# uga-ssrl/SSRLCV

Hardware: AMD Instinct MI355X
Metric: Mpix/s SIFT extract (+ Mmatches/s 128-D brute-force, see `matcher`) (higher is better)
Workload: dtype f32; 1 GPU; 2-view 4096x4096 pair per GPU (tools/scene.py pinhole views (PCG32 terrain + texture through Image::Camera)): SIFT_FeatureFactory::generateFeatures (sparse DoG path) on each image, pixels resident in HBM; images_per_gpu=2, parallelism=image-pair shard, library=release build (libssrlcv_hip_release.so)

## Files before the change

ssrlcv_amd/capi.py:

```python
import ctypes

import numpy as np
import torch

from . import _lib

LIB = _lib.load()

c_u32, c_f32, c_vp, c_sz, c_int = ctypes.c_uint32, ctypes.c_float, ctypes.c_void_p, ctypes.c_size_t, ctypes.c_int

OUT_DMATCH, OUT_UINT2_PAIR, OUT_MATCH = 0, 1, 2
_OUT_SIZE = {OUT_DMATCH: 48, OUT_UINT2_PAIR: 16, OUT_MATCH: 40}


class SsrlcvError(RuntimeError):
    pass


class MalformedPairList(SsrlcvError):
    """the device merge's input status word: an index out of range or a query matched twice in one pair"""


def check(rc):
    if rc != 0:
# ... 442 lines not shown


def math_eval(fn, a, b=None):
    a_d = torch.from_numpy(np.ascontiguousarray(a, dtype=np.float32)).cuda()
    b_d = None if b is None else torch.from_numpy(np.ascontiguousarray(b, dtype=np.float32)).cuda()
    out = torch.empty_like(a_d)
    check(LIB.ssrlcv_hip_math_eval(c_int(fn), ptr(a_d), ptr(b_d), ptr(out), c_sz(a_d.numel()), stream_ptr()))
    return out.cpu().numpy()


class SiftPlan:

    def __init__(self, w, h, max_orientations=2, orientation_threshold=0.8, orientation_contrib_width=1.5,
                 descriptor_contrib_width=6.0, max_keypoints_per_octave=0, alloc=True):
        self.w, self.h = w, h
        p = SiftParams(max_orientations, orientation_threshold, orientation_contrib_width, descriptor_contrib_width,
                       max_keypoints_per_octave)
        self.handle = c_vp()
        check(LIB.ssrlcv_sift_plan_create(c_u32(w), c_u32(h), ctypes.byref(p), ctypes.byref(self.handle)))
        self.workspace_bytes = LIB.ssrlcv_sift_plan_workspace_bytes(self.handle)
        self.max_features = LIB.ssrlcv_sift_plan_max_features(self.handle)
        self.workspace = dev_bytes(self.workspace_bytes) if alloc else None
        self.features = dev_bytes(self.max_features * 152) if alloc else None
        self.num_features = torch.zeros(1, dtype=torch.int32, device="cuda") if alloc else None

    def __del__(self):
        if getattr(self, "handle", None) and LIB is not None:
            LIB.ssrlcv_sift_plan_destroy(self.handle)
            self.handle = None

    def set_stop_stage(self, stage):
        LIB.ssrlcv_sift_plan_set_stop_stage(self.handle, c_int(stage))

    def set_stage_event(self, event):
        handle = None
        if event is not None:
            event.record()
            handle = event.cuda_event
        self._stage_event = event
        check(LIB.ssrlcv_sift_plan_set_stage_event(self.handle, c_vp(handle) if handle is not None else None))

    def build_dog(self, pixels_d):
        check(LIB.ssrlcv_hip_sift_build_dog(self.handle, ptr(pixels_d), ptr(self.workspace), stream_ptr()))

    def describe(self):
        check(LIB.ssrlcv_hip_sift_describe(self.handle, ptr(self.workspace), ptr(self.features),
                                           ptr(self.num_features), stream_ptr()))

    def stage(self, stage):
        check(LIB.ssrlcv_hip_sift_stage(self.handle, ptr(self.workspace), c_int(stage), ptr(self.features),
                                        ptr(self.num_features), stream_ptr()))

    def extract(self, pixels_d):
        check(LIB.ssrlcv_hip_sift_extract(self.handle, ptr(pixels_d), ptr(self.workspace), ptr(self.features),
                                          ptr(self.num_features), stream_ptr()))

    def count(self):
        mask = c_u32(0)
        rc = LIB.ssrlcv_sift_plan_overflow(self.handle, ptr(self.workspace), ctypes.byref(mask), stream_ptr())
        if mask.value:
            raise SsrlcvError("key-point capacity exceeded in octaves %s" % [o for o in range(4) if mask.value >> o & 1])
        check(rc)
        return int(self.num_features.item())

    def overflow_mask(self):
        mask = c_u32(0)
        LIB.ssrlcv_sift_plan_overflow(self.handle, ptr(self.workspace), ctypes.byref(mask), stream_ptr())
        return mask.value

    def level(self, kind, octave, blur):
        data, mm = c_vp(), c_vp()
        w, h = c_u32(), c_u32()
        check(LIB.ssrlcv_sift_plan_level(self.handle, ptr(self.workspace), c_int(kind), c_int(octave), c_int(blur),
                                         ctypes.byref(data), ctypes.byref(w), ctypes.byref(h), ctypes.byref(mm)))
        torch.cuda.synchronize()
        base = self.workspace.data_ptr()
        off = data.value - base
        n = w.value * h.value
        lvl = self.workspace[off: off + 4 * n].view(torch.float32).cpu().numpy().reshape(h.value, w.value).copy()
        moff = mm.value - base
        mmv = self.workspace[moff: moff + 8].view(torch.float32).cpu().numpy().copy()
        return lvl, (float(mmv[0]), float(mmv[1]))

    def keypoints(self, octave, dtype):
        lst, idx = c_vp(), c_vp()
        check(LIB.ssrlcv_sift_plan_keypoints(self.handle, ptr(self.workspace), c_int(octave), ctypes.byref(lst),
                                             ctypes.byref(idx)))
        torch.cuda.synchronize()
        base = self.workspace.data_ptr()
        ioff = idx.value - base
        state = self.workspace[ioff: ioff + 32].view(torch.int32).cpu().numpy().copy()
        n = int(state[5]) if int(state[6]) else 0
        loff = lst.value - base
        kps = to_host(self.workspace[loff: loff + 32 * max(n, 1)], dtype, n)
        return kps, state[:6].copy(), int(state[7])

    def features_host(self, dtype):
        n = self.count()
        return to_host(self.features[: 152 * max(n, 1)], dtype, n)
```

ssrlcv_amd/csrc/keypoints.hip:

```cpp
#include <hip/hip_runtime.h>
#include <float.h>
#include <math.h>
#include <stdlib.h>
#include "compact.h"
#include "dev_switch.h"
#include "scan_lookback.h"
#include "device_math.h"
#include "sift_plan.h"
#include "ssrlcv_hip.h"

using svp::OctaveState;

namespace {

struct LevelSet {
  const float* lvl[svp::kGauss];
  const float* lvlMinMax;
  const float* minmax;
  const float2* polar;
  int w, h;
};

struct DogView {
  const float* lo;
// ... 168 lines not shown
  float hess[3][3], hinv[3][3] = {{0.0f, 0.0f, 0.0f}, {0.0f, 0.0f, 0.0f}, {0.0f, 0.0f, 0.0f}};
  float grad[3], temp[3], offset[3] = {0.0f, 0.0f, 0.0f};
  int bl = kp.blur;
  for (int attempt = 0; attempt < 5; ++attempt) {
    const auto Dl = src.view(bl - 1), Dm = src.view(bl), Du = src.view(bl + 1);
#define PM(yy, xx) Dm.norm((size_t)(yy) * W + (xx))
#define PL(yy, xx) Dl.norm((size_t)(yy) * W + (xx))
#define PU(yy, xx) Du.norm((size_t)(yy) * W + (xx))
    grad[0] = PM(ly, lx + 1) - PM(ly, lx - 1);
    grad[1] = PM(ly + 1, lx) - PM(ly - 1, lx);
    grad[2] = PU(ly, lx) - PL(ly, lx);
    float centre = PM(ly, lx);
    hess[0][0] = grad[0] - 2 * centre;
    hess[0][1] = (PM(ly + 1, lx + 1) - PM(ly - 1, lx + 1) - PM(ly + 1, lx - 1) + PM(ly - 1, lx - 1)) / 4.0f;
    hess[0][2] = (PU(ly, lx + 1) - PL(ly, lx + 1) - PU(ly, lx - 1) + PL(ly, lx - 1)) / 4.0f;
    hess[1][0] = hess[0][1];
    hess[1][1] = grad[1] - 2 * centre;
    hess[1][2] = (PU(ly + 1, lx) - PL(ly + 1, lx) - PU(ly - 1, lx) + PL(ly - 1, lx)) / 4.0f;
    hess[2][0] = hess[0][2];
    hess[2][1] = hess[1][2];
    hess[2][2] = grad[2] - 2 * centre;
#pragma unroll
    for (int r = 0; r < 3; ++r)
#pragma unroll
      for (int c = 0; c < 3; ++c) hess[r][c] *= -1.0f;
    sv::inverse3(hess, hinv);
#pragma unroll
    for (int r = 0; r < 3; ++r) {
      float val = 0;
#pragma unroll
      for (int c = 0; c < 3; ++c) val = __builtin_fmaf(hinv[r][c], grad[c], val);
      offset[r] = val;
    }
#pragma unroll
    for (int c = 0; c < 3; ++c) {
      float val = 0;
#pragma unroll
      for (int r = 0; r < 3; ++r) val = __builtin_fmaf(hess[r][c], grad[r], val);
      temp[c] = val;
    }
    if (fabsf(offset[0]) <= 0.5f && fabsf(offset[1]) <= 0.5f && fabsf(offset[2]) <= 0.5f) {
      kp.loc.x = (float)lx + offset[0];
      kp.loc.y = (float)ly + offset[1];
      lx = (int)roundf(kp.loc.x);
      ly = (int)roundf(kp.loc.y);
      kp.discard = (uint8_t)(lx <= 0 || ly <= 0 || lx >= W - 1 || ly >= H - 1);
      if (kp.discard) break;
      kp.intensity = PM(ly, lx) - (0.5f * ((temp[0] * grad[0]) + (temp[1] * grad[1]) + (temp[2] * grad[2])));
      kp.sigma = sigmaMin * sv_powf(mult, ((float)bl + offset[2]));
      if (fabsf(offset[2]) > 0.5) bl += (offset[2] > 0) ? 1 : -1;
      break;
    } else if (attempt == 4) {
      kp.discard = 1;
      break;
    } else {
      if (fabsf(offset[0]) > 0.5) lx += (offset[0] > 0) ? 1 : -1;
      if (fabsf(offset[1]) > 0.5) ly += (offset[1] > 0) ? 1 : -1;
      kp.loc.x = (float)lx;
      kp.loc.y = (float)ly;
      if (fabsf(offset[2]) > 0.5) bl += (offset[2] > 0) ? 1 : -1;
      if (bl >= numBlurs - 1 || bl <= 0 || lx <= 0 || ly <= 0 || lx >= W - 1 || ly >= H - 1) {
        kp.discard = 1;
        break;
      }
    }
#undef PM
#undef PL
#undef PU
  }
  kp.blur = bl;
}

__global__ __launch_bounds__(256) void k_refine(const OctaveState* st, ssrlcv_sskeypoint* kps, LevelSet L, float sigmaMin,
                                                float mult) {
  int n = st->hasExtrema ? st->n : 0;
  const PlanSource src{L};
  for (int gi = blockIdx.x * 256 + threadIdx.x; gi < n; gi += gridDim.x * 256) {
    ssrlcv_sskeypoint kp = kps[gi];
    refine_one(kp, L.w, L.h, svp::kDog, sigmaMin, mult, src);
    kps[gi] = kp;
  }
}

constexpr int kPolRows = 16;
struct PolarJobs {
  LevelSet L[svp::kOctaves];
  float2* out[svp::kOctaves];
  uint32_t start[svp::kOctaves + 1];
  uint32_t tilesX[svp::kOctaves];
};
#ifndef SSRLCV_NT_STORES
#define SSRLCV_NT_STORES 1
#endif
typedef float f32x2p __attribute__((ext_vector_type(2)));
__device__ __forceinline__ float polar_ld(const float* p) {
#if SSRLCV_NT_STORES
  return __builtin_nontemporal_load(p);
#else
  return *p;
#endif
}
__global__ __launch_bounds__(256) void k_polar(PolarJobs jobs) {
  __shared__ float s_n[kPolRows][256 + 2];
  int o = 0;
#pragma unroll
  for (int k = 1; k < svp::kOctaves; ++k)
    if (blockIdx.x >= jobs.start[k]) o = k;
  const LevelSet& L = jobs.L[o];
  float2* __restrict__ out = jobs.out[o];
  const uint32_t tile = blockIdx.x - jobs.start[o];
  const int tileX = (int)(tile % jobs.tilesX[o]), tileY = (int)(tile / jobs.tilesX[o]);
  const int W = L.w, H = L.h;
  const int x0 = tileX * 256, y0 = tileY * kPolRows;
  const int t = threadIdx.x, x = x0 + t;
  const int xc = x < W ? x : W - 1;
  const bool haloRole = t < 2 * kPolRows;
  const int hside = t & 1;
  int hx = hside ? x0 + 256 : x0 - 1;
  hx = hx < 0 ? 0 : (hx > W - 1 ? W - 1 : hx);
  int hy = y0 + (t >> 1);
  hy = hy > H - 1 ? H - 1 : hy;
  size_t rowOff[kPolRows + 2];
#pragma unroll
  for (int j = 0; j < kPolRows + 2; ++j) {
    int yy = y0 - 1 + j;
    yy = yy < 0 ? 0 : (yy > H - 1 ? H - 1 : yy);
    rowOff[j] = (size_t)yy * W + xc;
  }
  const size_t haloOff = (size_t)hy * W + hx;
  float nlo[kPolRows + 2], nloH = 0.0f;
  {
    const float mn = L.lvlMinMax[2];
    const sv::Divisor rg = sv::make_divisor(L.lvlMinMax[3] - mn);
    const float* __restrict__ g = L.lvl[1];
#pragma unroll
    for (int j = 0; j < kPolRows + 2; ++j) nlo[j] = sv::div_by(polar_ld(g + rowOff[j]) - mn, rg);
    if (haloRole) nloH = sv::div_by(g[haloOff] - mn, rg);
  }
  const int cl = x == 0 ? 1 : (x == W - 1 ? t - 1 : t);
  const int cr = x == 0 ? 3 : (x == W - 1 ? t + 1 : t + 2);
#pragma unroll 1
  for (int lvl = 1; lvl <= 3; ++lvl) {
    const float mn = L.lvlMinMax[2 * (lvl + 1)];
    const sv::Divisor rg = sv::make_divisor(L.lvlMinMax[2 * (lvl + 1) + 1] - mn);
    const float dmn = L.minmax[2 * lvl];
    const sv::Divisor drg = sv::make_divisor(L.minmax[2 * lvl + 1] - dmn);
    const float* __restrict__ g = L.lvl[lvl + 1];
    float v[kPolRows + 2];
#pragma unroll
    for (int j = 0; j < kPolRows + 2; ++j) {
      const float nhi = sv::div_by(polar_ld(g + rowOff[j]) - mn, rg);
      v[j] = sv::div_by((nhi - nlo[j]) - dmn, drg);
      nlo[j] = nhi;
    }
    if (lvl > 1) __syncthreads();
#pragma unroll
    for (int i = 0; i < kPolRows; ++i) s_n[i][t + 1] = v[i + 1];
    if (haloRole) {
      const float nhi = sv::div_by(g[haloOff] - mn, rg);
      s_n[t >> 1][hside ? 257 : 0] = sv::div_by((nhi - nloH) - dmn, drg);
      nloH = nhi;
    }
    __syncthreads();
    float2* __restrict__ lvlOut = out + (size_t)(lvl - 1) * svp::polar_level_stride(W, H);
    if (tile == 0) {
      if (t == 0) lvlOut[0] = make_float2(0.0f, 0.0f);
      for (int i = t; i < W + 1; i += 256) lvlOut[1 + (size_t)W * H + i] = make_float2(0.0f, 0.0f);
    }
    if (x < W) {
      float2* __restrict__ o = lvlOut + 1 + (size_t)y0 * W + x;
#pragma unroll
      for (int i = 0; i < kPolRows; ++i) {
        const int y = y0 + i;
        if (y >= H) break;
        float2 g2;
        g2.x = s_n[i][cr] - s_n[i][cl];
        const float up = y == 0 ? v[i + 3 < kPolRows + 2 ? i + 3 : kPolRows + 1] : (y == H - 1 ? v[i + 1] : v[i + 2]);
        const float dn = y == 0 ? v[i + 1] : (y == H - 1 ? v[i > 0 ? i - 1 : 0] : v[i]);
        g2.y = up - dn;
        float2 r;
        r.x = sqrtf((g2.x * g2.x) + (g2.y * g2.y));
        r.y = sv_atan2f(g2.y, g2.x);
#if SSRLCV_NT_STORES
        __builtin_nontemporal_store(f32x2p{r.x, r.y}, reinterpret_cast<f32x2p*>(o + (size_t)i * W));
#else
        o[(size_t)i * W] = r;
#endif
      }
    }
  }
}
typedef float f32x2 __attribute__((ext_vector_type(2)));
__device__ __forceinline__ int round_pos(float v) {
  int r;
  asm("v_cvt_rpi_i32_f32 %0, %1" : "=v"(r) : "v"(v));
  return r;
}

__device__ __forceinline__ float fmod_2pi_above(float v, float p) { return v >= p ? v - p : v; }
__device__ __forceinline__ float2 polar_px(const float2* __restrict__ pl, int W, int x, int y) {
  return pl[y * W + x];
}
__device__ __forceinline__ int round_coord(float v) {
  int r;
  asm("v_cvt_rpi_i32_f32 %0, %1" : "=v"(r) : "v"(v));
  return v == -0.5f ? -1 : r;
}

constexpr int kThetaChunk = 8;

struct RangeTable {
  uint32_t first[20], count[20], start[20];
  uint32_t total;
  uint32_t pad[3];
};
static_assert(sizeof(RangeTable) == 256, "tables sit at 256-byte strides in the plan's group block");
__device__ __constant__ const int kSegOrder[5] = {3, 2, 1, 4, 0};
__device__ __forceinline__ void build_ranges(const OctaveState* st, RangeTable* tab, int unitShift, uint32_t sel) {
  uint32_t pos = 0;
  for (int k = 0; k < 5; ++k) {
    const int seg = kSegOrder[k];
    for (int o = 0; o < svp::kOctaves; ++o) {
      const int r = k * 4 + o;
      uint32_t first = 0, count = 0;
      if (st[o].hasExtrema && ((sel >> (o * 5 + seg)) & 1u)) {
        const int lo = st[o].idx[seg], hi = seg < svp::kDog - 1 ? st[o].idx[seg + 1] : st[o].n;
        if (hi > lo) { first = (uint32_t)lo; count = (uint32_t)(hi - lo); }
      }
      tab->first[r] = first;
      tab->count[r] = count;
      tab->start[r] = pos;
      pos += (count + (1u << unitShift) - 1) >> unitShift;
    }
  }
  tab->total = pos;
}
__global__ void k_build_ranges(const OctaveState* st, RangeTable* tab, int unitShift, uint32_t sel) { build_ranges(st, tab, unitShift, sel); }
__global__ void k_book_and_desc_ranges(OctaveState* st, uint32_t* featBase, uint32_t* numFeatures, uint32_t maxFeatures, RangeTable* tab) {
  uint32_t tot = 0;
  for (int o = 0; o < svp::kOctaves; ++o) {
    featBase[o] = tot;
    tot += st[o].hasExtrema ? (uint32_t)st[o].n : 0u;
  }
  if (tot > maxFeatures) tot = maxFeatures;
  *numFeatures = tot;
  build_ranges(st, tab, 0, 0xFFFFFu);
}

constexpr int kOct0Groups = svp::kSampleGroups - 1;
struct GroupCtl {
  uint32_t segStart[svp::kDog];
  uint32_t totals[svp::kSampleGroups + 1];
  uint32_t groupSum[svp::kSampleGroups];
  uint32_t done[svp::kSampleGroups];
  uint32_t regular;
  uint32_t cut[2];
  uint32_t pad[32 - svp::kDog - 3 * svp::kSampleGroups - 4];
};
static_assert(sizeof(GroupCtl) == 128, "four of them + eight range tables fit the plan's 4 KB group block");
__device__ __forceinline__ bool blur_indices_regular(const OctaveState* st) {
  if (!st->hasExtrema) return true;
  bool ok = st->idx[0] == 0;
  for (int k = 1; k < svp::kDog; ++k) ok = ok && st->idx[k - 1] <= st->idx[k];
  return ok && st->idx[svp::kDog - 1] <= st->n;
}
__global__ void k_build_group_ranges(const OctaveState* st, RangeTable* tabs, GroupCtl* ctl, int unitShift, bool forceIrregular) {
  const bool reg = blur_indices_regular(st) && !forceIrregular;
  const uint32_t n0 = st[0].hasExtrema && st[0].n > 0 ? (uint32_t)st[0].n : 0u;
  ctl[0].regular = reg ? 1u : 0u;
  ctl[0].cut[0] = reg && n0 ? (uint32_t)st[0].idx[2] : n0;
  ctl[0].cut[1] = reg && n0 ? (uint32_t)st[0].idx[3] : n0;
  const uint32_t oct0 = 0x1Fu, rest = 0xFFFFFu & ~oct0;
// ... 37 lines not shown
  int r = 0;
#pragma unroll
  for (int k = 1; k < 20; ++k)
    if (tab->start[k] <= u) r = k;
  return r;
}

struct OctaveSet {
  LevelSet L[svp::kOctaves];
  const ssrlcv_sskeypoint* kps[svp::kOctaves];
  float pixelWidth[svp::kOctaves];
  float* thetas[svp::kOctaves];
  uint32_t* thetaCnt[svp::kOctaves];
  const void* consts[svp::kOctaves];
};

template <int MAXO, int LPKS>
__global__ __launch_bounds__(64) void k_thetas(const OctaveState* states, const RangeTable* tab, OctaveSet set, float lambda,
                                               float orientationThreshold) {
  constexpr int LANES = 1 << LPKS, PER_BLOCK = 64 >> LPKS, CW = kThetaChunk * LANES;
  __shared__ float s_hist[36][PER_BLOCK];
  if (blockIdx.x >= tab->total) return;
  const int range = __builtin_amdgcn_readfirstlane(range_of(tab, blockIdx.x));
  const int octave = range & 3, useg = kSegOrder[range >> 2];
  const LevelSet& L = set.L[octave];
  const float pixelWidth = set.pixelWidth[octave];
  const int t = threadIdx.x, sub = t & (LANES - 1), col = t >> LPKS;
  const float fsub2 = (float)(2 * sub);
  const uint32_t local = (blockIdx.x - tab->start[range]) * PER_BLOCK + (uint32_t)(t >> LPKS);
  const bool have = local < tab->count[range];
  const int gi = (int)(tab->first[range] + local);
  const float pi = SSRLCV_PI_F;
  const float rad10 = pi / 18.0f;
  const float inv10 = 1.0f / rad10;
  ssrlcv_sskeypoint kp;
  kp.loc.x = kp.loc.y = 0.0f;
  kp.sigma = 1.0f;
  if (have) kp = set.kps[octave][gi];
  const float kx = kp.loc.x, ky = kp.loc.y;
  const float windowWidth = ceilf(kp.sigma * 3.0f * lambda / pixelWidth);
  const float minx = kx - windowWidth, miny = ky - windowWidth, maxx = kx + windowWidth, maxy = ky + windowWidth;
  const bool inside = have && useg >= 1 && useg <= 3 &&
                      !(minx < 0.0f || miny < 0.0f || maxx >= (unsigned)(L.w - 1) || maxy >= (unsigned)(L.h - 1));
#pragma unroll
  for (int i = 0; i < 36 * PER_BLOCK / 64; ++i) (&s_hist[0][0])[i * 64 + t] = 0.0f;
  const float weight = 2.0f * lambda * lambda * kp.sigma * kp.sigma;
  const float rweight = 1.0f / weight;
  const int W = L.w;
  const size_t levelStride = svp::polar_level_stride(L.w, L.h);
  {
    const float2* base = L.polar + (size_t)(useg - 1) * levelStride;
    const __amdgpu_buffer_rsrc_t rsrc = __builtin_amdgcn_make_buffer_rsrc((void*)base, 0, (int)(uint32_t)(levelStride * 8), 0x00020000);
    typedef unsigned u32x4 __attribute__((ext_vector_type(4)));
    typedef unsigned u32x2 __attribute__((ext_vector_type(2)));
    struct Cursor { float x, y, ty2; unsigned rowoff; bool act; };
    Cursor cf;
    cf.x = minx;
    cf.y = miny;
    cf.ty2 = (miny - ky) * (miny - ky);
    cf.rowoff = (unsigned)round_pos(miny) * (unsigned)W + 1u;
    cf.act = inside;
    auto advance = [&](Cursor& c) {
      float xn = c.x + (float)CW;
      if (__any(c.act && !(c.x >= (float)CW))) {
        float ch = c.x;
#pragma unroll 8
        for (int i = 0; i < CW; ++i) ch += 1.0f;
        xn = c.x >= (float)CW ? xn : ch;
      }
      if (c.act) {
        if (xn <= maxx) {
          c.x = xn;
        } else {
          c.x = minx;
          c.y += 1.0f;
          if (!(c.y <= maxy)) c.act = false;
          const float ty = c.y - ky;
          c.ty2 = ty * ty;
          c.rowoff = (unsigned)round_pos(c.y) * (unsigned)W + 1u;
        }
      }
    };
    typedef u32x4 Chunk[kThetaChunk / 2];
    auto fetch = [&](const Cursor& c, Chunk& into) {
      if (!c.act) return;
      const unsigned off = (c.rowoff + (unsigned)round_pos(c.x)) * 8u + 16u * (unsigned)sub;
#pragma unroll
      for (int j = 0; j < kThetaChunk / 4; ++j) into[j] = __builtin_amdgcn_raw_buffer_load_b128(rsrc, (int)(off + 16u * LANES * j), 0, 0);
    };
    auto fetch_upper = [&](const Cursor& c, Chunk& into) {
      if (!c.act) return;
      const unsigned off = (c.rowoff + (unsigned)round_pos(c.x)) * 8u + 16u * (unsigned)sub;
#pragma unroll
      for (int j = kThetaChunk / 4; j < kThetaChunk / 2; ++j) into[j] = __builtin_amdgcn_raw_buffer_load_b128(rsrc, (int)(off + 16u * LANES * j), 0, 0);
    };
    auto wants_upper = [&](const Cursor& c) { return __any(c.act && c.x + (float)(CW / 2 - 1) <= maxx); };
    Chunk qa, qb;
    Cursor ca, cb;
#pragma unroll
    for (int j = 0; j < kThetaChunk / 2; ++j) qa[j] = qb[j] = u32x4{0u, 0u, 0u, 0u};
    ca = cf;
    fetch(cf, qa);
    if (wants_upper(cf)) fetch_upper(cf, qa);
    advance(cf);
    cb = cf;
    auto step = [&](Chunk& cur, const Cursor& cc, Chunk& nxt, Cursor& cn) __attribute__((always_inline)) {
      cn = cf;
      fetch(cf, nxt);
      if (wants_upper(cf)) fetch_upper(cf, nxt);
      advance(cf);
      float xs[kThetaChunk];
      float xlast = cc.x + (float)(CW - 1);
#pragma unroll
      for (int i = 0; i < kThetaChunk; ++i) xs[i] = cc.x + (fsub2 + (float)(((i >> 1) << (1 + LPKS)) | (i & 1)));
      if (__any(cc.act && !(cc.x >= (float)CW))) {
        float ch = cc.x;
        float xc[kThetaChunk];
#pragma unroll
        for (int sIdx = 0; sIdx < CW; ++sIdx) {
          const int q = (sIdx >> 1) & (LANES - 1), i = ((sIdx >> (1 + LPKS)) << 1) | (sIdx & 1);
          if (LANES == 1 || q == 0) xc[i] = ch;
          else xc[i] = sub == q ? ch : xc[i];
          if (sIdx + 1 < CW) ch += 1.0f;
        }
        const bool direct = cc.x >= (float)CW;
#pragma unroll
        for (int i = 0; i < kThetaChunk; ++i) xs[i] = direct ? xs[i] : xc[i];
        xlast = direct ? xlast : ch;
      }
      const float cty2 = cc.ty2;
      const unsigned crow = cc.rowoff;
      const bool cact = cc.act;
      const bool aligned = cc.x >= 4.0f && round_pos(xlast) == round_pos(cc.x) + (CW - 1);
      if (__any(cact && !aligned)) {
        if (cact && !aligned) {
#pragma unroll
          for (int i = 0; i < kThetaChunk; ++i) {
            u32x2 e = u32x2{0u, 0u};
            if (xs[i] <= maxx) e = __builtin_amdgcn_raw_buffer_load_b64(rsrc, (int)((crow + (unsigned)round_pos(xs[i])) * 8u), 0, 0);
            cur[i >> 1][(i & 1) * 2] = e[0];
            cur[i >> 1][(i & 1) * 2 + 1] = e[1];
          }
        }
      }
      auto weigh = [&](float ang, float xi, float& wgt, int& bin) {
        const float angle = fmod_2pi_above(ang + (2.0f * pi), 2.0f * pi);
        bin = (int)floorf(sv::exact_div3(angle, rad10, inv10));
        const float tx = xi - kx;
        wgt = sv::expf_nonpos(sv::exact_div5(-((tx * tx) + cty2), weight, rweight));
      };
      const bool upperHalf = __any(cact && xs[kThetaChunk / 2] <= maxx);
      float wg[kThetaChunk], mg[kThetaChunk];
      float* slot[kThetaChunk];
      auto weigh_half = [&](auto hc) __attribute__((always_inline)) {
        constexpr int i0 = decltype(hc)::value * (kThetaChunk / 2);
#pragma unroll
        for (int i = i0; i < i0 + kThetaChunk / 2; ++i) {
          const unsigned um = cur[i >> 1][(i & 1) * 2], ua = cur[i >> 1][(i & 1) * 2 + 1];
          int bin;
          weigh(__builtin_bit_cast(float, ua), xs[i], wg[i], bin);
          const bool counts = cact && xs[i] <= maxx && (unsigned)bin < 36u;
          slot[i] = &s_hist[counts ? bin : 0][col];
          mg[i] = counts ? __builtin_bit_cast(float, um) : 0.0f;
        }
      };
      auto vote_half = [&](auto hc) __attribute__((always_inline)) {
        constexpr int j0 = decltype(hc)::value * (kThetaChunk / 4);
#pragma unroll
        for (int j = j0; j < j0 + kThetaChunk / 4; ++j) {
#pragma unroll
          for (int q = 0; q < LANES; ++q) {
            if (LANES == 1 || sub == q) {
              const float h0 = *slot[2 * j], h1 = *slot[2 * j + 1];
              const float n0 = fmaf(mg[2 * j], wg[2 * j], h0);
              const float n1 = fmaf(mg[2 * j + 1], wg[2 * j + 1], slot[2 * j + 1] == slot[2 * j] ? n0 : h1);
              *slot[2 * j] = n0;
              *slot[2 * j + 1] = n1;
            }
// ... 246 lines not shown
          const float mmag = m == 0 ? magA : m == 1 ? magB : m == 2 ? magC : magD;
#pragma unroll 1
          for (int cell = 0; cell < 16; ++cell) {
            const int ci = lane & 15;
            (void)ci;
            const float hx0 = ((float)(cell >> 2) * 0.5f - 0.75f) * windowWidth, hy0 = ((float)(cell & 3) * 0.5f - 0.75f) * windowWidth;
            const float rx = (hx0 * c) + (hy0 * s), ry = (-hx0 * s) + (hy0 * c);
            float hx = fabsf(rx - mcx), hy = fabsf(ry - mcy);
            if (hx <= binWidth && hy <= binWidth) {
              hx = hx / binWidth;
              hy = hy / binWidth;
              for (int k = 0; k < 8; ++k) {
                float angle = fabsf(mang - ((float)k * rad45));
                if (angle < rad45) {
                  angle /= rad45;
                  const float temp = (1.0f - hx) * (1.0f - hy) * (1.0f - angle) * mmag;
                  atomicAdd(bins + (cell * 8 + k) * kDescCopies + copy, vote_u32(temp));
                }
              }
            }
          }
        }
      }
    }
    __builtin_amdgcn_wave_barrier();
    unsigned t0 = 0u, t1 = 0u;
#pragma unroll
    for (int cpy = 0; cpy < kDescCopies; ++cpy) {
      t0 += bins[lane * kDescCopies + cpy];
      t1 += bins[(lane + 64) * kDescCopies + cpy];
    }
    float v0 = (float)t0, v1 = (float)t1;
    float sq = sqrtf(sv::wave_sum((v0 * v0) + (v1 * v1)));
    v0 = v0 / sq;
    v1 = v1 / sq;
    if (v0 > 0.2f) v0 = 0.2f;
    if (v1 > 0.2f) v1 = 0.2f;
    sq = sqrtf(sv::wave_sum((v0 * v0) + (v1 * v1)));
    {
      int b0 = lane, b1 = lane + 64;
      int o0 = (((b0 >> 3) & 3) * 4 + (b0 >> 5)) * 8 + (b0 & 7);
      int o1 = (((b1 >> 3) & 3) * 4 + (b1 >> 5)) * 8 + (b1 & 7);
      s_bytes[wave][o0] = (uint8_t)roundf(255.0f * v0 / sq);
      s_bytes[wave][o1] = (uint8_t)roundf(255.0f * v1 / sq);
    }
    __builtin_amdgcn_wave_barrier();
    const uint32_t fi = featBase[octave] + (uint32_t)gi;
    if (fi < maxFeatures) {
      ssrlcv_sift_feature* f = features + fi;
      if (lane < 16) *reinterpret_cast<uint2*>(&f->values[lane * 8]) = *reinterpret_cast<const uint2*>(&s_bytes[wave][lane * 8]);
      if (lane == 16) {
        f->parent = -1;
        reinterpret_cast<int*>(f)[1] = 0;
        f->theta = kp.theta;
        f->sigma = kp.sigma;
        f->loc.x = kp.loc.x * pixelWidth;
        f->loc.y = kp.loc.y * pixelWidth;
      }
    }
    __builtin_amdgcn_wave_barrier();
  }
}

LevelSet make_levels(const ssrlcv_sift_plan* plan, char* ws, int o) {
  LevelSet L;
  const svp::OctavePlan& oc = plan->oct[o];
  for (int b = 0; b < svp::kGauss; ++b) L.lvl[b] = (const float*)(ws + plan->off_gauss[o][b]);
  L.lvlMinMax = (const float*)(ws + plan->off_minmax) + (size_t)o * 2 * (svp::kGauss + svp::kDog);
  L.minmax = L.lvlMinMax + 2 * svp::kGauss;
  L.polar = (const float2*)(ws + oc.off_polar);
  L.w = (int)oc.w;
  L.h = (int)oc.h;
  return L;
}

void launch_polar(const ssrlcv_sift_plan* plan, char* ws, hipStream_t st, int oFirst = 0, int oLast = svp::kOctaves - 1) {
  PolarJobs jobs;
  uint32_t pos = 0;
  for (int o = 0; o < svp::kOctaves; ++o) {
    const svp::OctavePlan& oc = plan->oct[o];
    jobs.L[o] = make_levels(plan, ws, o);
    jobs.out[o] = (float2*)(ws + oc.off_polar);
    jobs.start[o] = pos;
    jobs.tilesX[o] = (oc.w + 255) / 256;
    if (o >= oFirst && o <= oLast) pos += jobs.tilesX[o] * ((oc.h + kPolRows - 1) / kPolRows);
  }
  jobs.start[svp::kOctaves] = pos;
  hipLaunchKernelGGL(k_polar, dim3(pos), dim3(256), 0, st, jobs);
}

}
namespace svp {
void launch_polar_octave(const ssrlcv_sift_plan* plan, char* ws, int octave, hipStream_t st) {
  PolarJobs jobs;
  const svp::OctavePlan& oc = plan->oct[octave];
  const uint32_t tilesX = (oc.w + 255) / 256, tiles = tilesX * ((oc.h + kPolRows - 1) / kPolRows);
  for (int o = 0; o < svp::kOctaves; ++o) {
    jobs.L[o] = make_levels(plan, ws, octave);
    jobs.out[o] = (float2*)(ws + oc.off_polar);
    jobs.tilesX[o] = tilesX;
    jobs.start[o] = o <= octave ? 0u : tiles;
  }
  jobs.start[svp::kOctaves] = tiles;
  hipLaunchKernelGGL(k_polar, dim3(tiles), dim3(256), 0, st, jobs);
}
}
namespace {
hipError_t run_discard(OctaveState* st, const ssrlcv_sskeypoint* src, ssrlcv_sskeypoint* dst, uint32_t cap,
                       uint32_t* words, hipStream_t stream) {
  const OctaveState* cst = st;
  auto keyfn = [=] __device__(uint32_t i) -> uint32_t {
    if (!cst->hasExtrema || (int)i >= cst->n) return 0u;
    if (src[i].discard) return 0u;
    return 1u << segment_of(cst, (int)i);
  };
  auto emit = [=] __device__(uint32_t i, int, uint32_t d) { dst[d] = src[i]; };
  uint32_t* totals = nullptr;
  auto post = [=] __device__(const uint32_t* tot) { book_discard(st, tot); };
  return svc::partition<svp::kDog, 8>(cap, keyfn, emit, words, &totals, stream, &st->n, 1u, post);
}

constexpr unsigned kWaveKernelOversubscription = 16;
inline unsigned list_blocks(uint32_t cap) {
  unsigned b = (cap + 255) / 256;
  return b > 1024 ? 1024 : b;
}

}

extern "C" {

int ssrlcv_sift_plan_keypoints(const ssrlcv_sift_plan* plan, void* workspace, int octave, ssrlcv_sskeypoint** list,
                               int** blurIndices_dev) {
  if (!plan || !workspace || octave < 0 || octave >= svp::kOctaves) return SSRLCV_ERR_INVALID_ARG;
  char* ws = (char*)workspace;
  if (list) *list = (ssrlcv_sskeypoint*)(ws + (plan->listInB[octave] ? plan->oct[octave].off_kpB : plan->oct[octave].off_kpA));
  if (blurIndices_dev) *blurIndices_dev = (int*)(ws + plan->off_state + sizeof(OctaveState) * octave);
  return SSRLCV_OK;
}

int ssrlcv_sift_plan_overflow(const ssrlcv_sift_plan* plan, const void* workspace, uint32_t* octaveMask,
                              ssrlcv_stream_t stream) {
  if (!plan || !workspace || !octaveMask) return SSRLCV_ERR_INVALID_ARG;
  OctaveState st[svp::kOctaves];
  SSRLCV_HIP_TRY(hipMemcpyAsync(st, (const char*)workspace + plan->off_state, sizeof st, hipMemcpyDeviceToHost,
                                (hipStream_t)stream));
  SSRLCV_HIP_TRY(hipStreamSynchronize((hipStream_t)stream));
  uint32_t m = 0;
  for (int o = 0; o < svp::kOctaves; ++o)
    if (st[o].overflow) m |= 1u << o;
  *octaveMask = m;
  return m ? SSRLCV_ERR_CAPACITY : SSRLCV_OK;
}

}
namespace {

struct ListCtx {
  const ssrlcv_sift_plan* plan;
  const svp::OctavePlan* oc;
  int o;
  hipStream_t s;
  OctaveState* st;
  LevelSet L;
  ssrlcv_sskeypoint *A, *B;
  uint8_t* flags;
  uint32_t* words;
  uint32_t cap;
  ssrlcv_sskeypoint* cur() const { return plan->listInB[o] ? B : A; }
  ssrlcv_sskeypoint* oth() const { return plan->listInB[o] ? A : B; }
  void flip() const { plan->listInB[o] ^= 1; }
};
ListCtx make_ctx(const ssrlcv_sift_plan* plan, char* ws, int o, hipStream_t s) {
  ListCtx c;
  c.plan = plan;
  c.oc = &plan->oct[o];
  c.o = o;
  c.s = s;
  c.st = (OctaveState*)(ws + plan->off_state) + o;
  c.L = make_levels(plan, ws, o);
  c.A = (ssrlcv_sskeypoint*)(ws + c.oc->off_kpA);
  c.B = (ssrlcv_sskeypoint*)(ws + c.oc->off_kpB);
  c.flags = (uint8_t*)(ws + c.oc->off_flags);
  c.words = (uint32_t*)(ws + c.oc->off_part);
  c.cap = c.oc->cap;
  return c;
}
// ... 1070 lines not shown
```

ssrlcv_amd/csrc/pyramid.hip:

```cpp
#include <hip/hip_runtime.h>
#include <map>
#include <mutex>
#include <float.h>
#include <math.h>
#include <new>
#include <stdlib.h>
#include <string.h>
#include "dev_switch.h"
#include "device_math.h"
#include "sift_plan.h"
#include "ssrlcv_hip.h"

namespace {

__device__ __forceinline__ int sym_coord(int i, int l) {
  int ll = 2 * l;
  if (__builtin_expect(i < -ll || i >= ll, 0)) i = (i + ll) % ll;
  if (i < 0) i += ll;
  return (i > l - 1) ? ll - 1 - i : i;
}

__device__ __forceinline__ int mirror_into(int i, int l, int R) {
  if (l < 64) return sym_coord(i, l);
  i = i > l - 1 + R ? l - 1 + R : i;
// ... 1805 lines not shown
    uint32_t cap = params->maxKeyPointsPerOctave ? params->maxKeyPointsPerOctave : (uint32_t)(P / 16);
    if (cap < 4096) cap = 4096;
    oc.cap = cap;
    oc.off_kpA = take((size_t)cap * sizeof(ssrlcv_sskeypoint));
    oc.off_kpB = take((size_t)cap * sizeof(ssrlcv_sskeypoint));
    oc.off_theta = take((size_t)cap * svp::kMaxOrient * sizeof(float));
    oc.off_thetaCnt = take((size_t)cap * sizeof(uint32_t));
    size_t words = (size_t)3 * 4 * ((P + 8191) / 8192) + 16 +
                   (size_t)svp::kDog * 4 * (((size_t)cap * svp::kMaxOrient + 2047) / 2048) + 16;
    oc.off_part = take(words * 4);
    oc.off_featBase = take(256);
    oc.off_descConst = take((size_t)cap * 32);
    maxFeat += cap;
    if (o + 1 < svp::kOctaves) {
      ow /= 2;
      oh /= 2;
      pixelWidth *= 2.0f;
      for (int b = 0; b < svp::kGauss; ++b) sigmas[b] *= mulX;
    }
  }
  p->off_extremaCounts = take(256);
  p->off_dogPartial = take(sizeof(float) * 2 * svp::kDog * svp::kDogMaxWaves * svp::kOctaves);
  p->off_groups = take(4096);
  p->total = off;
  p->maxFeatures = maxFeat;
  *out = p;
  return SSRLCV_OK;
}

void ssrlcv_sift_plan_destroy(ssrlcv_sift_plan* plan) {
  if (!plan) return;
  if (plan->async) {
    svp::PlanAsync* a = plan->async;
    (void)hipEventDestroy(a->fork);
    for (hipEvent_t e : a->join) (void)hipEventDestroy(e);
    for (hipEvent_t e : a->convDone) (void)hipEventDestroy(e);
    for (hipEvent_t e : a->dogDone) (void)hipEventDestroy(e);
    for (hipEvent_t e : a->polarDone) (void)hipEventDestroy(e);
    for (hipEvent_t e : a->binDone) (void)hipEventDestroy(e);
    (void)hipEventDestroy(a->expandFork);
    (void)hipEventDestroy(a->groupFork);
    for (hipEvent_t e : a->groupExpanded) (void)hipEventDestroy(e);
    for (hipEvent_t e : a->groupReady) (void)hipEventDestroy(e);
    for (hipEvent_t e : a->expandJoin) (void)hipEventDestroy(e);
    for (auto& lv : a->levelDone)
      for (hipEvent_t e : lv) (void)hipEventDestroy(e);
    delete a;
  }
  delete plan;
}
size_t ssrlcv_sift_plan_workspace_bytes(const ssrlcv_sift_plan* plan) { return plan ? plan->total : 0; }
uint32_t ssrlcv_sift_plan_max_features(const ssrlcv_sift_plan* plan) { return plan ? plan->maxFeatures : 0; }
void ssrlcv_sift_plan_set_stop_stage(ssrlcv_sift_plan* plan, int stage) { if (plan) plan->stopStage = stage; }
int ssrlcv_sift_plan_set_stage_event(ssrlcv_sift_plan* plan, void* event) {
  if (!plan) return SSRLCV_ERR_INVALID_ARG;
  plan->stageEvent = (hipEvent_t)event;
  return SSRLCV_OK;
}

int ssrlcv_sift_plan_level(const ssrlcv_sift_plan* plan, void* workspace, int kind, int octave, int blur, float** data,
                           uint32_t* w, uint32_t* h, float** minmax_dev) {
  if (!plan || !workspace || octave < 0 || octave >= svp::kOctaves) return SSRLCV_ERR_INVALID_ARG;
  char* ws = (char*)workspace;
  const svp::OctavePlan& oc = plan->oct[octave];
  float* mm = (float*)(ws + plan->off_minmax) + (size_t)octave * 2 * (svp::kGauss + svp::kDog);
  if (kind == 0) {
    if (blur < 0 || blur >= svp::kDog) return SSRLCV_ERR_INVALID_ARG;
    if (((size_t)oc.w * oc.h) % 4) return SSRLCV_ERR_UNSUPPORTED;
    SSRLCV_HIP_TRY(hipDeviceSynchronize());
    const float* lv[svp::kGauss];
    float* dogs[svp::kDog];
    float* scratch = (float*)(ws + plan->off_in0);
    for (int b = 0; b < svp::kGauss; ++b) lv[b] = (const float*)(ws + plan->off_gauss[octave][b]);
    for (int b = 0; b < svp::kDog; ++b) dogs[b] = scratch;
    int rc = launch_dog(lv, mm, oc.w, oc.h, dogs, nullptr, blur, blur + 1, 1024, nullptr, nullptr);
    if (rc) return rc;
    SSRLCV_HIP_TRY(hipDeviceSynchronize());
    if (data) *data = scratch;
    if (minmax_dev) *minmax_dev = mm + 2 * (svp::kGauss + blur);
  } else if (kind == 1) {
    if (blur < 0 || blur >= svp::kGauss) return SSRLCV_ERR_INVALID_ARG;
    if (data) *data = (float*)(ws + plan->off_gauss[octave][blur]);
    if (minmax_dev) *minmax_dev = mm + 2 * blur;
  } else {
    return SSRLCV_ERR_INVALID_ARG;
  }
  if (w) *w = oc.w;
  if (h) *h = oc.h;
  return SSRLCV_OK;
}

int ssrlcv_hip_sift_build_dog(const ssrlcv_sift_plan* plan, const uint8_t* pixels, void* workspace,
                              ssrlcv_stream_t stream) {
  if (!plan || !pixels || !workspace) return SSRLCV_ERR_INVALID_ARG;
  hipStream_t st = (hipStream_t)stream;
  char* ws = (char*)workspace;
  float* mmAll = (float*)(ws + plan->off_minmax);
  const int pairs = (svp::kGauss + svp::kDog) * svp::kOctaves;
  svp::PlanAsync* as = svp::plan_async(plan);
  hipStream_t sd = as ? as->table : st;
  const auto& sw = svdev::sw();
  const bool overlapOctaves = !sw.noOctaveOverlap;
  const int overlapFrom = sw.octaveOverlapFrom;
  const int deferDog0 = sw.dogx0After;
  const bool earlyPolar = as && plan->fusedCall && plan->stopStage >= 6 && sw.earlyPolar;
  plan->polarInFlight = 0;
  plan->chain0InFlight = 0;
  if (earlyPolar) {
    SSRLCV_HIP_TRY(hipEventRecord(as->fork, st));
    SSRLCV_HIP_TRY(hipStreamWaitEvent(as->polar, as->fork, 0));
  }
  hipLaunchKernelGGL(k_init_minmax, dim3(1), dim3(64), 0, st, mmAll, pairs);
  float* in = (float*)(ws + plan->off_in0);
  int rc;
  bool fuseUpsample = false;
  if (plan->padMode == 1) {
    const uint32_t pw = plan->W + 2 * plan->padX, ph = plan->H + 2 * plan->padY;
    uint8_t* padded = (uint8_t*)(ws + plan->off_pad);
    hipLaunchKernelGGL(k_add_border<uint8_t>, dim3((pw + 255) / 256, ph), dim3(256), 0, st, pixels, plan->W, plan->H, padded,
                       plan->padX, plan->padY);
    rc = ssrlcv_hip_upsample2x_u8(padded, pw, ph, in, stream);
  } else if (plan->padMode == 2) {
    float* up = (float*)(ws + plan->off_pad);
    rc = ssrlcv_hip_upsample2x_u8(pixels, plan->W, plan->H, up, stream);
    hipLaunchKernelGGL(k_add_border<float>, dim3((plan->oct[0].w + 255) / 256, plan->oct[0].h), dim3(256), 0, st, up,
                       2 * plan->W, 2 * plan->H, in, plan->padX, plan->padY);
  } else if (upsample_fusable(plan->oct[0].w, plan->oct[0].h, plan->oct[0].taps[0])) {
    rc = 0;
    fuseUpsample = true;
  } else {
    rc = ssrlcv_hip_upsample2x_u8(pixels, plan->W, plan->H, in, stream);
  }
  if (rc) return rc;
  float* nextIn[3] = {(float*)(ws + plan->off_in1), (float*)(ws + plan->off_in2), (float*)(ws + plan->off_in1)};
  const float firstNoise = (float)(svp::kNoiseThreshold * 0.8);
  const int phased = sw.phased;
  if (as && phased > 0) {
    const int ahead = phased - 1;
    const float* octIn = in;
    for (int o = 0; o < svp::kOctaves; ++o) {
      const svp::OctavePlan& oc = plan->oct[o];
      float* mm = mmAll + (size_t)o * 2 * (svp::kGauss + svp::kDog);
      const float* src = octIn;
      for (int b = 0; b < 4; ++b) {
        float* dst = (float*)(ws + plan->off_gauss[o][b]);
        bool binned = false;
        rc = launch_conv(src, dst, nullptr, oc.w, oc.h, oc.taps[b], oc.weights[b], mm + 2 * b, st,
                         (fuseUpsample && o == 0 && b == 0) ? pixels : nullptr, (b == 3 && o + 1 < svp::kOctaves) ? nextIn[o] : nullptr, &binned);
        if (rc) return rc;
        src = dst;
        if (b == 3 && o + 1 < svp::kOctaves) {
          if (!binned) {
            rc = ssrlcv_hip_bin2x(dst, oc.w, oc.h, nextIn[o], (ssrlcv_stream_t)st);
            if (rc) return rc;
          }
          octIn = nextIn[o];
        }
      }
      SSRLCV_HIP_TRY(hipEventRecord(as->binDone[o], st));
    }
    for (int o = 0; o < svp::kOctaves; ++o) {
      const svp::OctavePlan& oc = plan->oct[o];
      float* mm = mmAll + (size_t)o * 2 * (svp::kGauss + svp::kDog);
      const hipStream_t sb = o == 0 ? as->table : (o == 1 ? as->chain : st);
      const int gate = o + ahead < svp::kOctaves ? o + ahead : svp::kOctaves - 1;
      if (sb != st) SSRLCV_HIP_TRY(hipStreamWaitEvent(sb, as->binDone[gate], 0));
// ... 114 lines not shown
```

Before: 3585 Mpix/s.

## Rewrite polar gradient kernel as single-wave row-streaming strips with buffer loads

The polar (magnitude/angle) kernel moves from 256-thread tiles with an LDS halo exchange to one 64-lane wave per vertical strip segment. Each wave streams down its rows with a software-pipelined load queue of configurable depth, uses buffer loads and stores, and gets horizontal neighbours through ds_bpermute instead of shared memory and barriers. Strip indices are also swizzled across blocks. The theta fetch path now redirects unwanted chunk loads to an out-of-range offset so they return zero instead of reading memory. A debug accessor for the polar table is added as well. The risks are more register pressure, fewer threads per block, and subtle correctness at image borders.

```diff
diff --git a/ssrlcv_amd/capi.py b/ssrlcv_amd/capi.py
--- a/ssrlcv_amd/capi.py
+++ b/ssrlcv_amd/capi.py
@@ -548,6 +548,17 @@
         mmv = self.workspace[moff: moff + 8].view(torch.float32).cpu().numpy().copy()
         return lvl, (float(mmv[0]), float(mmv[1]))
 
+    def polar_table(self, octave, level):
+        data = c_vp()
+        w, h = c_u32(), c_u32()
+        check(LIB.ssrlcv_sift_plan_level(self.handle, ptr(self.workspace), c_int(2), c_int(octave), c_int(level),
+                                         ctypes.byref(data), ctypes.byref(w), ctypes.byref(h), None))
+        torch.cuda.synchronize()
+        off = data.value - self.workspace.data_ptr()
+        n = w.value * h.value
+        raw = self.workspace[off - 8: off + 8 * (n + w.value + 1)].view(torch.float32).cpu().numpy().reshape(-1, 2).copy()
+        return raw[1: 1 + n].reshape(h.value, w.value, 2), raw[0], raw[1 + n:]
+
     def keypoints(self, octave, dtype):
         lst, idx = c_vp(), c_vp()
         check(LIB.ssrlcv_sift_plan_keypoints(self.handle, ptr(self.workspace), c_int(octave), ctypes.byref(lst),
diff --git a/ssrlcv_amd/csrc/keypoints.hip b/ssrlcv_amd/csrc/keypoints.hip
--- a/ssrlcv_amd/csrc/keypoints.hip
+++ b/ssrlcv_amd/csrc/keypoints.hip
@@ -274,112 +274,195 @@
   }
 }
 
-constexpr int kPolRows = 16;
+#ifndef SSRLCV_POLAR_SEG
+#define SSRLCV_POLAR_SEG 64
+#endif
+#ifndef SSRLCV_POLAR_DEPTH
+#define SSRLCV_POLAR_DEPTH 3
+#endif
+#ifndef SSRLCV_POLAR_COLS
+#define SSRLCV_POLAR_COLS 2
+#endif
+constexpr int kPolCols = SSRLCV_POLAR_COLS, kPolStrip = 64 * kPolCols, kPolSeg = SSRLCV_POLAR_SEG, kPolDepth = SSRLCV_POLAR_DEPTH;
+static_assert(kPolSeg >= 3 && kPolDepth >= 1, "a segment holds a whole vertical stencil");
 struct PolarJobs {
   LevelSet L[svp::kOctaves];
   float2* out[svp::kOctaves];
   uint32_t start[svp::kOctaves + 1];
-  uint32_t tilesX[svp::kOctaves];
+  uint32_t strips[svp::kOctaves];
 };
-#ifndef SSRLCV_NT_STORES
-#define SSRLCV_NT_STORES 1
+__device__ __forceinline__ void polar_item(uint32_t item, uint32_t strips, uint32_t& sx, uint32_t& sy) {
+  sx = item % strips;
+  sy = item / strips;
+  if ((strips & 7u) == 0u) {
+    const uint32_t per = strips >> 3, q = item >> 3;
+    sx = (item & 7u) * per + q % per;
+    sy = q / per;
+  }
+}
+#ifdef SSRLCV_POLAR_WAVES
+__attribute__((amdgpu_waves_per_eu(SSRLCV_POLAR_WAVES)))
 #endif
-typedef float f32x2p __attribute__((ext_vector_type(2)));
-__device__ __forceinline__ float polar_ld(const float* p) {
-#if SSRLCV_NT_STORES
-  return __builtin_nontemporal_load(p);
-#else
-  return *p;
-#endif
-}
-__global__ __launch_bounds__(256) void k_polar(PolarJobs jobs) {
-  __shared__ float s_n[kPolRows][256 + 2];
+__global__ __launch_bounds__(64) void k_polar(PolarJobs jobs) {
   int o = 0;
 #pragma unroll
   for (int k = 1; k < svp::kOctaves; ++k)
     if (blockIdx.x >= jobs.start[k]) o = k;
   const LevelSet& L = jobs.L[o];
   float2* __restrict__ out = jobs.out[o];
-  const uint32_t tile = blockIdx.x - jobs.start[o];
-  const int tileX = (int)(tile % jobs.tilesX[o]), tileY = (int)(tile / jobs.tilesX[o]);
+  const uint32_t item = blockIdx.x - jobs.start[o];
+  uint32_t sx, sy;
+  polar_item(item, jobs.strips[o], sx, sy);
   const int W = L.w, H = L.h;
-  const int x0 = tileX * 256, y0 = tileY * kPolRows;
-  const int t = threadIdx.x, x = x0 + t;
-  const int xc = x < W ? x : W - 1;
-  const bool haloRole = t < 2 * kPolRows;
-  const int hside = t & 1;
-  int hx = hside ? x0 + 256 : x0 - 1;
-  hx = hx < 0 ? 0 : (hx > W - 1 ? W - 1 : hx);
-  int hy = y0 + (t >> 1);
-  hy = hy > H - 1 ? H - 1 : hy;
-  size_t rowOff[kPolRows + 2];
-#pragma unroll
-  for (int j = 0; j < kPolRows + 2; ++j) {
-    int yy = y0 - 1 + j;
-    yy = yy < 0 ? 0 : (yy > H - 1 ? H - 1 : yy);
-    rowOff[j] = (size_t)yy * W + xc;
-  }
-  const size_t haloOff = (size_t)hy * W + hx;
-  float nlo[kPolRows + 2], nloH = 0.0f;
-  {
-    const float mn = L.lvlMinMax[2];
-    const sv::Divisor rg = sv::make_divisor(L.lvlMinMax[3] - mn);
-    const float* __restrict__ g = L.lvl[1];
-#pragma unroll
-    for (int j = 0; j < kPolRows + 2; ++j) nlo[j] = sv::div_by(polar_ld(g + rowOff[j]) - mn, rg);
-    if (haloRole) nloH = sv::div_by(g[haloOff] - mn, rg);
-  }
-  const int cl = x == 0 ? 1 : (x == W - 1 ? t - 1 : t);
-  const int cr = x == 0 ? 3 : (x == W - 1 ? t + 1 : t + 2);
+  const int x0 = (int)sx * kPolStrip, y0 = (int)sy * kPolSeg;
+  const int y1 = y0 + kPolSeg < H ? y0 + kPolSeg : H;
+  const int lane = threadIdx.x;
+  const int ya = y0 == 0 ? -2 : (y0 - 1 < H - 3 ? y0 - 1 : H - 3);
+  const int yb = y1 < H ? y1 : H - 1;
+  const int firstMain = y0 == 0 ? 2 : y0 + 1;
+  unsigned col[kPolCols], colc[kPolCols];
+#pragma unroll
+  for (int k = 0; k < kPolCols; ++k) {
+    col[k] = x0 + lane + 64 * k;
+    colc[k] = col[k] < (unsigned)W ? col[k] : (unsigned)(W - 1);
+  }
+  const bool haloLane = lane == 0 || lane == 63;
+  int hx = lane == 0 ? x0 - 1 : x0 + kPolStrip;
+  const unsigned hxc = (unsigned)(hx < 0 ? 0 : (hx > W - 1 ? W - 1 : hx));
+  const bool firstStrip = x0 == 0, lastStrip = x0 + kPolStrip >= W;
+  const int rotUp = ((lane + 63) & 63) * 4, rotDn = ((lane + 1) & 63) * 4;
+  float gmn[4], dmn[3];
+  sv::Divisor grg[4], drg[3];
+#pragma unroll
+  for (int l = 0; l < 4; ++l) {
+    gmn[l] = L.lvlMinMax[2 * (l + 1)];
+    grg[l] = sv::make_divisor(L.lvlMinMax[2 * (l + 1) + 1] - gmn[l]);
+  }
+#pragma unroll
+  for (int l = 0; l < 3; ++l) {
+    dmn[l] = L.minmax[2 * (l + 1)];
+    drg[l] = sv::make_divisor(L.minmax[2 * (l + 1) + 1] - dmn[l]);
+  }
+  const size_t levelStride = svp::polar_level_stride(W, H);
+  typedef unsigned u32x2 __attribute__((ext_vector_type(2)));
+  __amdgpu_buffer_rsrc_t rin[4], rout[3];
+#pragma unroll
+  for (int l = 0; l < 4; ++l) rin[l] = __builtin_amdgcn_make_buffer_rsrc((void*)L.lvl[l + 1], 0, (int)((uint32_t)W * (uint32_t)H * 4u), 0x00020000);
+#pragma unroll
+  for (int l = 0; l < 3; ++l) rout[l] = __builtin_amdgcn_make_buffer_rsrc((void*)(out + (size_t)l * levelStride), 0, (int)(uint32_t)(levelStride * 8), 0x00020000);
+  if (item == 0) {
 #pragma unroll 1
-  for (int lvl = 1; lvl <= 3; ++lvl) {
-    const float mn = L.lvlMinMax[2 * (lvl + 1)];
-    const sv::Divisor rg = sv::make_divisor(L.lvlMinMax[2 * (lvl + 1) + 1] - mn);
-    const float dmn = L.minmax[2 * lvl];
-    const sv::Divisor drg = sv::make_divisor(L.minmax[2 * lvl + 1] - dmn);
-    const float* __restrict__ g = L.lvl[lvl + 1];
-    float v[kPolRows + 2];
-#pragma unroll
-    for (int j = 0; j < kPolRows + 2; ++j) {
-      const float nhi = sv::div_by(polar_ld(g + rowOff[j]) - mn, rg);
-      v[j] = sv::div_by((nhi - nlo[j]) - dmn, drg);
-      nlo[j] = nhi;
-    }
-    if (lvl > 1) __syncthreads();
-#pragma unroll
-    for (int i = 0; i < kPolRows; ++i) s_n[i][t + 1] = v[i + 1];
-    if (haloRole) {
-      const float nhi = sv::div_by(g[haloOff] - mn, rg);
-      s_n[t >> 1][hside ? 257 : 0] = sv::div_by((nhi - nloH) - dmn, drg);
-      nloH = nhi;
-    }
-    __syncthreads();
-    float2* __restrict__ lvlOut = out + (size_t)(lvl - 1) * svp::polar_level_stride(W, H);
-    if (tile == 0) {
-      if (t == 0) lvlOut[0] = make_float2(0.0f, 0.0f);
-      for (int i = t; i < W + 1; i += 256) lvlOut[1 + (size_t)W * H + i] = make_float2(0.0f, 0.0f);
-    }
-    if (x < W) {
-      float2* __restrict__ o = lvlOut + 1 + (size_t)y0 * W + x;
-#pragma unroll
-      for (int i = 0; i < kPolRows; ++i) {
-        const int y = y0 + i;
-        if (y >= H) break;
-        float2 g2;
-        g2.x = s_n[i][cr] - s_n[i][cl];
-        const float up = y == 0 ? v[i + 3 < kPolRows + 2 ? i + 3 : kPolRows + 1] : (y == H - 1 ? v[i + 1] : v[i + 2]);
-        const float dn = y == 0 ? v[i + 1] : (y == H - 1 ? v[i > 0 ? i - 1 : 0] : v[i]);
-        g2.y = up - dn;
-        float2 r;
-        r.x = sqrtf((g2.x * g2.x) + (g2.y * g2.y));
-        r.y = sv_atan2f(g2.y, g2.x);
-#if SSRLCV_NT_STORES
-        __builtin_nontemporal_store(f32x2p{r.x, r.y}, reinterpret_cast<f32x2p*>(o + (size_t)i * W));
-#else
-        o[(size_t)i * W] = r;
-#endif
-      }
-    }
+    for (int l = 0; l < 3; ++l) {
+      float2* lvlOut = out + (size_t)l * levelStride;
+      if (lane == 0) lvlOut[0] = make_float2(0.0f, 0.0f);
+      for (int i = lane; i < W + 1; i += 64) lvlOut[1 + (size_t)W * H + i] = make_float2(0.0f, 0.0f);
+    }
+  }
+  struct RowIn { float g[4][kPolCols + 1]; };
+  auto request = [&](int i, RowIn& r) __attribute__((always_inline)) {
+    if (i > yb) return;
+    const int row = (int)((uint32_t)(i < 0 ? -i : i) * (uint32_t)W * 4u);
+#pragma unroll
+    for (int l = 0; l < 4; ++l) {
+#pragma unroll
+      for (int k = 0; k < kPolCols; ++k) r.g[l][k] = __builtin_bit_cast(float, __builtin_amdgcn_raw_buffer_load_b32(rin[l], (int)(colc[k] * 4u), row, 2));
+      float hv = 0.0f;
+      if (haloLane) hv = __builtin_bit_cast(float, __builtin_amdgcn_raw_buffer_load_b32(rin[l], (int)(hxc * 4u), row, 0));
+      r.g[l][kPolCols] = hv;
+    }
+  };
+  float v0[3][kPolCols], v1[3][kPolCols], gx1[3][kPolCols];
+#pragma unroll
+  for (int l = 0; l < 3; ++l)
+#pragma unroll
+    for (int k = 0; k < kPolCols; ++k) v0[l][k] = v1[l][k] = gx1[l][k] = 0.0f;
+  auto process = [&](const RowIn& r, int y) __attribute__((always_inline)) {
+    float nlo[kPolCols + 1];
+#pragma unroll
+    for (int j = 0; j < kPolCols + 1; ++j) nlo[j] = sv::div_by(r.g[0][j] - gmn[0], grg[0]);
+    const bool mainRow = y >= firstMain && y - 1 < y1;
+    const bool topRow = y == 0, bottomRow = y == H - 1 && y1 == H;
+    const int nEmit = (mainRow ? 1 : 0) + ((topRow || bottomRow) ? 1 : 0);
+#pragma unroll
+    for (int l = 0; l < 3; ++l) {
+      float v[kPolCols + 1];
+#pragma unroll
+      for (int j = 0; j < kPolCols + 1; ++j) {
+        const float nhi = sv::div_by(r.g[l + 1][j] - gmn[l + 1], grg[l + 1]);
+        v[j] = sv::div_by((nhi - nlo[j]) - dmn[l], drg[l]);
+        nlo[j] = nhi;
+      }
+      float gx2[kPolCols], nxt[kPolCols], prv[kPolCols];
+#pragma unroll
+      for (int k = 0; k < kPolCols; ++k) {
+        nxt[k] = __builtin_bit_cast(float, __builtin_amdgcn_ds_bpermute(rotDn, __builtin_bit_cast(int, v[k])));
+        prv[k] = __builtin_bit_cast(float, __builtin_amdgcn_ds_bpermute(rotUp, __builtin_bit_cast(int, v[k])));
+      }
+#pragma unroll
+      for (int k = 0; k < kPolCols; ++k) {
+        const float right = lane == 63 ? (k < kPolCols - 1 ? nxt[k < kPolCols - 1 ? k + 1 : k] : v[kPolCols]) : nxt[k];
+        const float left = lane == 0 ? (k > 0 ? prv[k > 0 ? k - 1 : k] : v[kPolCols]) : prv[k];
+        gx2[k] = right - left;
+      }
+      if (firstStrip) {
+        const float g1 = __builtin_bit_cast(float, __builtin_amdgcn_ds_bpermute(rotDn, __builtin_bit_cast(int, gx2[0])));
+        gx2[0] = lane == 0 ? g1 : gx2[0];
+      }
+      if (lastStrip) {
+#pragma unroll
+        for (int k = 0; k < kPolCols; ++k) {
+          const float g1 = __builtin_bit_cast(float, __builtin_amdgcn_ds_bpermute(rotUp, __builtin_bit_cast(int, gx2[k])));
+          gx2[k] = col[k] == (unsigned)(W - 1) ? g1 : gx2[k];
+        }
+      }
+#pragma unroll 1
+      for (int e = 0; e < nEmit; ++e) {
+        const bool mainNow = mainRow && e == 0;
+        const int yo = mainNow ? y - 1 : y;
+        const int orow = (int)((uint32_t)yo * (uint32_t)W * 8u);
+#pragma unroll
+        for (int k = 0; k < kPolCols; ++k) {
+          const float gx = mainNow ? gx1[l][k] : gx2[k];
+          const float gy = topRow ? v0[l][k] - v[k] : v[k] - v0[l][k];
+          const float mag = sqrtf((gx * gx) + (gy * gy));
+          const float ang = sv_atan2f(gy, gx);
+          if (col[k] < (unsigned)W)
+            __builtin_amdgcn_raw_buffer_store_b64(u32x2{__builtin_bit_cast(unsigned, mag), __builtin_bit_cast(unsigned, ang)}, rout[l],
+                                                  (int)(col[k] * 8u + 8u), orow, 2);
+          __builtin_amdgcn_sched_barrier(0);
+        }
+      }
+#pragma unroll
+      for (int k = 0; k < kPolCols; ++k) {
+        v0[l][k] = v1[l][k];
+        v1[l][k] = v[k];
+        gx1[l][k] = gx2[k];
+      }
+    }
+  };
+  static_assert(kPolDepth <= 4, "four turns are written out");
+  RowIn buf[kPolDepth] = {};
+  auto turn = [&](auto dc, int y, bool first) __attribute__((always_inline)) {
+    constexpr int d = decltype(dc)::value;
+    if constexpr (d < kPolDepth) {
+      if (first) {
+        request(y + d, buf[d]);
+      } else if (y + d <= yb) {
+        process(buf[d], y + d);
+        request(y + d + kPolDepth, buf[d]);
+      }
+    }
+  };
+  turn(std::integral_constant<int, 0>{}, ya, true);
+  turn(std::integral_constant<int, 1>{}, ya, true);
+  turn(std::integral_constant<int, 2>{}, ya, true);
+  turn(std::integral_constant<int, 3>{}, ya, true);
+#pragma unroll 1
+  for (int y = ya; y <= yb; y += kPolDepth) {
+    turn(std::integral_constant<int, 0>{}, y, false);
+    turn(std::integral_constant<int, 1>{}, y, false);
+    turn(std::integral_constant<int, 2>{}, y, false);
+    turn(std::integral_constant<int, 3>{}, y, false);
   }
 }
 typedef float f32x2 __attribute__((ext_vector_type(2)));
@@ -583,18 +666,19 @@
       }
     };
     typedef u32x4 Chunk[kThetaChunk / 2];
-    auto fetch = [&](const Cursor& c, Chunk& into) {
+    const unsigned pastTable = (unsigned)(levelStride * 8);
+    auto fetch_pieces = [&](const Cursor& c, Chunk& into, auto half) __attribute__((always_inline)) {
       if (!c.act) return;
+      constexpr int j0 = decltype(half)::value * (kThetaChunk / 4);
       const unsigned off = (c.rowoff + (unsigned)round_pos(c.x)) * 8u + 16u * (unsigned)sub;
 #pragma unroll
-      for (int j = 0; j < kThetaChunk / 4; ++j) into[j] = __builtin_amdgcn_raw_buffer_load_b128(rsrc, (int)(off + 16u * LANES * j), 0, 0);
+      for (int j = j0; j < j0 + kThetaChunk / 4; ++j) {
+        const bool wanted = c.x + (fsub2 + (float)(2 * LANES * j - 1)) <= maxx;
+        into[j] = __builtin_amdgcn_raw_buffer_load_b128(rsrc, (int)(wanted ? off + 16u * LANES * j : pastTable), 0, 0);
+      }
     };
-    auto fetch_upper = [&](const Cursor& c, Chunk& into) {
-      if (!c.act) return;
-      const unsigned off = (c.rowoff + (unsigned)round_pos(c.x)) * 8u + 16u * (unsigned)sub;
-#pragma unroll
-      for (int j = kThetaChunk / 4; j < kThetaChunk / 2; ++j) into[j] = __builtin_amdgcn_raw_buffer_load_b128(rsrc, (int)(off + 16u * LANES * j), 0, 0);
-    };
+    auto fetch = [&](const Cursor& c, Chunk& into) __attribute__((always_inline)) { fetch_pieces(c, into, std::integral_constant<int, 0>{}); };
+    auto fetch_upper = [&](const Cursor& c, Chunk& into) __attribute__((always_inline)) { fetch_pieces(c, into, std::integral_constant<int, 1>{}); };
     auto wants_upper = [&](const Cursor& c) { return __any(c.act && c.x + (float)(CW / 2 - 1) <= maxx); };
     Chunk qa, qb;
     Cursor ca, cb;
@@ -1007,11 +1091,11 @@
     jobs.L[o] = make_levels(plan, ws, o);
     jobs.out[o] = (float2*)(ws + oc.off_polar);
     jobs.start[o] = pos;
-    jobs.tilesX[o] = (oc.w + 255) / 256;
-    if (o >= oFirst && o <= oLast) pos += jobs.tilesX[o] * ((oc.h + kPolRows - 1) / kPolRows);
+    jobs.strips[o] = (oc.w + kPolStrip - 1) / kPolStrip;
+    if (o >= oFirst && o <= oLast) pos += jobs.strips[o] * ((oc.h + kPolSeg - 1) / kPolSeg);
   }
   jobs.start[svp::kOctaves] = pos;
-  hipLaunchKernelGGL(k_polar, dim3(pos), dim3(256), 0, st, jobs);
+  hipLaunchKernelGGL(k_polar, dim3(pos), dim3(64), 0, st, jobs);
 }
 
 }
@@ -1019,15 +1103,15 @@
 void launch_polar_octave(const ssrlcv_sift_plan* plan, char* ws, int octave, hipStream_t st) {
   PolarJobs jobs;
   const svp::OctavePlan& oc = plan->oct[octave];
-  const uint32_t tilesX = (oc.w + 255) / 256, tiles = tilesX * ((oc.h + kPolRows - 1) / kPolRows);
+  const uint32_t strips = (oc.w + kPolStrip - 1) / kPolStrip, tiles = strips * ((oc.h + kPolSeg - 1) / kPolSeg);
   for (int o = 0; o < svp::kOctaves; ++o) {
     jobs.L[o] = make_levels(plan, ws, octave);
     jobs.out[o] = (float2*)(ws + oc.off_polar);
-    jobs.tilesX[o] = tilesX;
+    jobs.strips[o] = strips;
     jobs.start[o] = o <= octave ? 0u : tiles;
   }
   jobs.start[svp::kOctaves] = tiles;
-  hipLaunchKernelGGL(k_polar, dim3(tiles), dim3(256), 0, st, jobs);
+  hipLaunchKernelGGL(k_polar, dim3(tiles), dim3(64), 0, st, jobs);
 }
 }
 namespace {
diff --git a/ssrlcv_amd/csrc/pyramid.hip b/ssrlcv_amd/csrc/pyramid.hip
--- a/ssrlcv_amd/csrc/pyramid.hip
+++ b/ssrlcv_amd/csrc/pyramid.hip
@@ -1911,6 +1911,10 @@
     if (blur < 0 || blur >= svp::kGauss) return SSRLCV_ERR_INVALID_ARG;
     if (data) *data = (float*)(ws + plan->off_gauss[octave][blur]);
     if (minmax_dev) *minmax_dev = mm + 2 * blur;
+  } else if (kind == 2) {
+    if (blur < 1 || blur > 3) return SSRLCV_ERR_INVALID_ARG;
+    if (data) *data = (float*)(ws + oc.off_polar) + 2 * ((size_t)(blur - 1) * svp::polar_level_stride(oc.w, oc.h) + 1);
+    if (minmax_dev) *minmax_dev = nullptr;
   } else {
     return SSRLCV_ERR_INVALID_ARG;
   }
```

After: 3355 Mpix/s. 6.4% lower.
